# bytedance/DeepSolid

Hardware: AMD Instinct MI355X
Metric: local-energy evals/sec (higher is better)
Workload: dtype f64; 1 GPU; bcc_li 24 e- (12,12), total_energy primal (E_kin forward-Laplacian + Ewald), default detnet ((256,32),)*3, 8 dets; batch_per_gpu=4096, global_batch=4096, parallelism=walker-dp1

## Files before the change

### deepsolid_amd/_lib.py

```python
import ctypes as C
import os

_HERE = os.path.dirname(os.path.abspath(__file__))
LIB_PATH = os.environ.get('DEEPSOLID_HIP_LIB') or os.path.join(_HERE, 'libdeepsolid_hip.so')

DS_MAX_LAYERS = 8
DS_MAX_SYM = 6
_PD = C.POINTER(C.c_double)


class SystemDesc(C.Structure):
    _fields_ = [
        ('dtype', C.c_int32), ('n_up', C.c_int32), ('n_dn', C.c_int32), ('n_atoms_prim', C.c_int32),
        ('prim_atoms', _PD), ('prim_a', C.c_double * 9), ('sim_a', C.c_double * 9), ('n_sym', C.c_int32),
        ('prim_AV', C.c_double * (DS_MAX_SYM * 3)), ('prim_BV', C.c_double * (DS_MAX_SYM * 3)),
        ('sim_AV', C.c_double * (DS_MAX_SYM * 3)), ('sim_BV', C.c_double * (DS_MAX_SYM * 3)),
        ('n_layers', C.c_int32), ('hidden_single', C.c_int32 * DS_MAX_LAYERS),
        ('hidden_double', C.c_int32 * DS_MAX_LAYERS), ('n_det', C.c_int32), ('distance_type', C.c_int32),
        ('envelope_type', C.c_int32), ('full_det', C.c_int32), ('use_last_layer', C.c_int32),
        ('bias_orbitals', C.c_int32), ('klist_up', _PD), ('klist_dn', _PD),
        ('n_atoms_sim', C.c_int32), ('sim_atoms', _PD), ('sim_charges', _PD), ('dist_mode', C.c_int32),
        ('n_g', C.c_int32), ('gpoints', _PD), ('gweight', _PD), ('ion_exp_re', _PD), ('ion_exp_im', _PD),
        ('ewald_alpha', C.c_double), ('ee_const', C.c_double), ('ei_const', C.c_double), ('ii_total', C.c_double),
    ]
# ... 16 lines not shown
        ('shell_l', _PI), ('shell_nprim', _PI), ('exps', _PD), ('coefs', _PD), ('n_k', C.c_int32), ('kpts', _PD),
        ('n_images', C.c_int32), ('images', _PD), ('n_up', C.c_int32), ('n_dn', C.c_int32), ('nocc_up', _PI), ('nocc_dn', _PI),
        ('mo_up', _PD), ('mo_dn', _PD),
    ]


class EcpDesc(C.Structure):
    _PI = C.POINTER(C.c_int32)
    _fields_ = [
        ('a', C.c_double * 9), ('n_atoms', C.c_int32), ('atoms', _PD), ('atom_species', _PI), ('n_species', C.c_int32),
        ('n_l', _PI), ('r_cut_loc', _PD), ('r_cut_nl', _PD), ('term_offset', _PI), ('term_n', _PI), ('term_zeta', _PD),
        ('term_c', _PD), ('n_quad', C.c_int32),
    ]


_VP = C.c_void_p


def _dmc_step_sig(n_lead, n_noise, n_out, ecp):
    step = [C.c_int64, C.c_int] + [C.c_double] * 5 + [C.c_int, C.c_int, C.c_uint64, C.c_uint64]
    return (C.c_int, [_VP] * n_lead + step + [_VP] * n_noise + ([C.c_int64] if ecp else []) + [C.c_int] + [_VP] * n_out +
            ([C.POINTER(C.c_int)] if ecp else []) + [_VP, C.c_int64, _VP])


SIGNATURES = {
    'ds_device_widths': (C.c_int, [C.POINTER(C.c_int32), C.POINTER(C.c_int32), C.c_int32, C.c_int32, C.c_int32, C.c_int32,
                                   C.POINTER(C.c_int32), C.POINTER(C.c_int32), C.POINTER(C.c_int32), C.POINTER(C.c_int32)]),
    'ds_system_create': (C.c_int, [C.POINTER(SystemDesc), C.POINTER(_VP)]),
    'ds_system_destroy': (None, [_VP]),
    'ds_last_error': (C.c_char_p, []),
    'ds_param_count': (C.c_int64, [_VP]),
    'ds_int8_layers': (C.c_int, [_VP]),
    'ds_pair_recompute_layers': (C.c_int, [_VP, C.c_int]),
    'ds_param_layout': (C.c_int, [_VP, C.POINTER(ParamBlock), C.c_int]),
    'ds_workspace_bytes': (C.c_int64, [_VP, C.c_int64]),
    'ds_logpsi': (C.c_int, [_VP, _VP, _VP, C.c_int64, _VP, _VP, _VP, C.c_int64, _VP]),
    'ds_logpsi_grad': (C.c_int, [_VP, _VP, _VP, C.c_int64, _VP, _VP, _VP, _VP, C.c_int64, _VP]),
    'ds_vjp_workspace_bytes': (C.c_int64, [_VP, C.c_int64]),
    'ds_logpsi_vjp': (C.c_int, [_VP, _VP, _VP, C.c_int64, _VP, _VP, _VP, _VP, _VP, C.c_int64, _VP]),
    'ds_pretrain_workspace_bytes': (C.c_int64, [_VP, C.c_int64]),
    'ds_pretrain_loss_vjp': (C.c_int, [_VP, _VP, _VP, C.c_int64, _VP, _VP, _VP, _VP, _VP, C.c_int64, _VP]),
    'ds_kfac_block_count': (C.c_int, [_VP]),
    'ds_kfac_layout': (C.c_int, [_VP, C.POINTER(KfacBlock), C.c_int]),
    'ds_kfac_workspace_bytes': (C.c_int64, [_VP, C.c_int64]),
    'ds_kfac_factors': (C.c_int, [_VP, _VP, _VP, C.c_int64, _VP, _VP, _VP, C.c_int64, _VP]),
    'ds_kfac_step_workspace_bytes': (C.c_int64, [_VP]),
    'ds_kfac_inverses': (C.c_int, [_VP, _VP, C.c_double, C.c_double, _VP, _VP, C.c_int64, _VP]),
    'ds_kfac_precondition': (C.c_int, [_VP, _VP, _VP, _VP, _VP, _VP, C.c_int64, _VP]),
    'ds_kfac_inverses_sized_workspace_bytes': (C.c_int64, [C.c_int, C.POINTER(C.c_int32), C.POINTER(C.c_int32)]),
    'ds_kfac_inverses_sized': (C.c_int, [C.c_int, C.c_int, C.POINTER(C.c_int32), C.POINTER(C.c_int32), C.POINTER(C.c_int32), _VP,
                                        C.c_double, C.c_double, _VP, _VP, C.c_int64, _VP]),
    'ds_jacobian_workspace_bytes': (C.c_int64, [_VP, C.c_int64]),
    'ds_logpsi_jacobian': (C.c_int, [_VP, _VP, _VP, C.c_int64, _VP, C.c_int64, _VP, _VP, _VP, C.c_int64, _VP]),
    'ds_minsr_gram_workspace_bytes': (C.c_int64, [C.c_int64, C.c_int64]),
    'ds_minsr_gram': (C.c_int, [C.c_int, _VP, C.c_int64, C.c_int64, C.c_int64, _VP, _VP, C.c_int64, _VP]),
    'ds_minsr_matvec_workspace_bytes': (C.c_int64, [C.c_int, C.c_int64, C.c_int64]),
    'ds_minsr_matvec': (C.c_int, [C.c_int, C.c_int, _VP, C.c_int64, C.c_int64, C.c_int64, _VP, _VP, _VP, C.c_int64, _VP]),
    'ds_minsr_solve_workspace_bytes': (C.c_int64, [C.c_int64, C.c_int64]),
    'ds_minsr_solve': (C.c_int, [C.c_int64, C.c_int64, C.c_double, C.c_double, _VP, _VP, _VP, _VP, C.c_int64, _VP]),
    'ds_orbitals': (C.c_int, [_VP, _VP, _VP, C.c_int64, _VP, _VP, _VP, C.c_int64, _VP]),
    'ds_ewald': (C.c_int, [_VP, _VP, C.c_int64, _VP, _VP]),
    'ds_local_energy': (C.c_int, [_VP, _VP, _VP, C.c_int64, _VP, _VP, _VP, _VP, _VP, C.c_int64, _VP]),
    'ds_enforce_pbc': (C.c_int, [_PD, C.c_int, _VP, C.c_int64, _VP, _VP, _VP]),
    'ds_observables_workspace_bytes': (C.c_int64, [C.c_int64, C.c_int]),
    'ds_observables': (C.c_int, [_PD, C.c_int, _VP, C.c_int64, C.c_int64, C.POINTER(C.c_int32), C.c_int, C.c_int, _VP, _VP,
                                 C.c_int64, _VP]),
# ... 86 lines not shown
```

### deepsolid_amd/csrc/ds_api.hip

```cpp
#include <cstdarg>

#include "ds_host.h"
#include "ds_tiles.h"

namespace ds {
#define DS_DECL(p) const TileOps<double>* tile_ops_f64_p##p(int); const TileOps<float>* tile_ops_f32_p##p(int);
DS_DECL(0) DS_DECL(1) DS_DECL(2) DS_DECL(3) DS_DECL(4)
#undef DS_DECL
template <> const TileOps<double>* tile_ops<double>(int st) {
    const TileOps<double>* (*parts[])(int) = {tile_ops_f64_p0, tile_ops_f64_p1, tile_ops_f64_p2, tile_ops_f64_p3, tile_ops_f64_p4};
    for (auto f : parts)
        if (const TileOps<double>* o = f(st)) return o;
    return nullptr;
}
template <> const TileOps<float>* tile_ops<float>(int st) {
    const TileOps<float>* (*parts[])(int) = {tile_ops_f32_p0, tile_ops_f32_p1, tile_ops_f32_p2, tile_ops_f32_p3, tile_ops_f32_p4};
    for (auto f : parts)
        if (const TileOps<float>* o = f(st)) return o;
    return nullptr;
}
}

namespace ds {
namespace host {
// ... 309 lines not shown
        hipMemcpy(s->blob32, h32.data(), h32.size() * sizeof(float), hipMemcpyHostToDevice) != hipSuccess) {
        ds_system_destroy(s);
        return fail("upload of the system tables failed");
    }
    relocate<double>(s->sd, (const double*)s->blob64);
    relocate<float>(s->sf, (const float*)s->blob32);
    build_layouts(s);
    {
        int h1max = 0;
        for (int l = 0; l <= s->sd.n_layers; ++l) h1max = std::max(h1max, s->sd.h1[l]);
        if (hipMalloc(&s->lr_w0t, (size_t)h1max * 64 * sizeof(double)) != hipSuccess) {
            ds_system_destroy(s);
            return fail("hipMalloc of the low-rank layer's weight table failed");
        }
    }
    {
        hipDeviceProp_t prop;
        int devid = 0;
        if (hipGetDevice(&devid) == hipSuccess && hipGetDeviceProperties(&prop, devid) == hipSuccess && prop.multiProcessorCount > 0)
            s->n_cu = prop.multiProcessorCount;
    }
    if (hipMalloc((void**)&s->clk_dev, 1024 * sizeof(unsigned long long)) != hipSuccess ||
        hipMemset(s->clk_dev, 0, 1024 * sizeof(unsigned long long)) != hipSuccess) {
        ds_system_destroy(s);
        return fail("hipMalloc of the clock-probe counters failed");
    }
    s->det_valu = getenv("DS_DET_VALU") != nullptr;
    if (const char* e = getenv("DS_VAL_NB")) { const int v = atoi(e); s->val_nb = (v == 1 || v == 2 || v == 4) ? v : 0; }
    s->no_lu_wave = getenv("DS_NO_LU_WAVE") != nullptr;
    s->use_lr = getenv("DS_NO_LOWRANK") == nullptr;
    s->use_pm_skip = getenv("DS_NO_PM_SKIP") == nullptr;
    s->use_pair_expand = getenv("DS_NO_PAIR_EXPAND") == nullptr;
    s->use_pair_recompute = getenv("DS_NO_PAIR_RECOMPUTE") == nullptr;
    s->use_g4 = getenv("DS_NO_G4") == nullptr;
    s->use_i8 = getenv("DS_I8") != nullptr && getenv("DS_NO_I8") == nullptr;
    s->use_ldsb = getenv("DS_NO_LDSB") == nullptr;
    s->use_pair_fuse = getenv("DS_NO_PAIR_FUSE") == nullptr;
    s->use_i8_val = getenv("DS_NO_I8_VAL") == nullptr;
    for (int l = 0; l < DS_MAX_LAYERS; ++l) s->i8_prepped[l] = ~(uint64_t)0;
    if (const char* e = getenv("DS_I8_VAL_MIN_TILES")) s->val_i8_min_tiles = atoll(e);
    if (const char* e = getenv("DS_DBG")) s->dbg = atoi(e);
    s->use_wide = getenv("DS_NO_WIDE") == nullptr;
    s->wide_all = getenv("DS_WIDE_ALL") != nullptr;
    {
        const size_t bytes = i8_planes_bytes(s);
        if (bytes && hipMalloc(&s->i8_wp, bytes) != hipSuccess) {
            ds_system_destroy(s);
            return fail("hipMalloc of the int8 layer's weight planes failed");
        }
    }
    if (const char* e = getenv("DS_CHUNK_WALKERS")) s->chunk_cap = std::min<int64_t>(65535, std::max<int64_t>(1, atol(e)));
    *out = s;
    return 0;
}

void ds_system_destroy(ds_system* s) {
    if (!s) return;
    if (s->clk_dev) (void)hipFree(s->clk_dev);
    if (s->lr_w0t) (void)hipFree(s->lr_w0t);
    if (s->i8_wp) (void)hipFree(s->i8_wp);
    if (s->blob64) (void)hipFree(s->blob64);
    if (s->blob32) (void)hipFree(s->blob32);
    delete s;
}

int64_t ds_param_count(const ds_system* s) { return s ? s->nparams : -1; }
// ... 100 lines not shown
```

### deepsolid_amd/csrc/ds_chain.hip

```cpp
#include "ds_host.h"
#include "ds_tiles.h"

namespace ds {
namespace host {

template <typename T> inline unsigned m2_split(int K2, int N) {
    unsigned z = 1;
    while (z < 8 && K2 % (2 * z) == 0 && (size_t)(K2 / z) * 5 * N * sizeof(T) > 8192) z *= 2;
    return z;
}

enum Stop { STOP_NONE = 0, STOP_G0, STOP_G1, STOP_G2, STOP_G3, STOP_H2_0, STOP_H2_1, STOP_H2_2, STOP_MEAN0, STOP_Q,
            STOP_MOUT, STOP_MINV, STOP_DETS, STOP_TR };

template <typename T> struct DumpReq { int stop; T* out; int64_t cap; int64_t written; };

template <typename T>
int copy_out(DumpReq<T>* dr, const T* src, size_t n, hipStream_t st) {
    size_t m = std::min<size_t>(n, (size_t)dr->cap);
    HIP_OK(hipMemcpyAsync(dr->out, src, m * sizeof(T), hipMemcpyDeviceToDevice, st));
    dr->written = (int64_t)m;
    return 0;
}

enum class LayerKind {
    Dense,
    DenseRes,
    L0Stats,
    L0Epi9Means,
    LowRank1,
    Int8
};
struct PairPlan {
    bool res, res_sep;
    bool expand;
    bool write_out;
    unsigned xz; int EW, NW; size_t xlds;
    bool recompute_prev;
};
struct LayerPlan {
    LayerKind kind;
    bool res_sep;
    bool wide;
    bool pm_mask;
    bool pm_unwritten;
    int prof_kind;
    PairPlan pair;
};
enum class OrbKind { Orb3, Wide, Ldsb, Gemm };
template <typename T> struct ChainPlan {
    const ds::TileOps<T>* to;
    bool lr_on;
    int lr_nc;
    int g4;
    LayerPlan layer[DS_MAX_LAYERS];
    OrbKind orb[2];
    int count(LayerKind k, int n_layers) const {
        int n = 0;
        for (int l = 0; l < n_layers; ++l) n += layer[l].kind == k ? 1 : 0;
        return n;
    }
};

template <typename T>
int plan_chain(const ds_system* s, bool dump, ChainPlan<T>* p) {
    const ds::SysDev<double>& S = s->sd;
    const ds::TileOps<T>* to = p->to = ds::tile_ops<T>(S.P / 16);
    if (!to) return fail("no kernel instance for %d slot tiles (N = %d electrons)", S.P / 16, S.N);
    const int ST = to->ST;
    const bool wide = s->use_wide && to->gemm_wide != nullptr;
    auto gemm_wide = [&](int epi) { return wide && (s->wide_all || ds::gemm_wide_faster<T>(epi)); };
    const int K0loc = S.h1[0] + S.nch * S.h2[0], K0sh = S.nch * S.h1[0];
    p->lr_nc = std::max(2, (K0loc + K0sh + 4 + 15) / 16);
    p->lr_on = !dump && s->use_lr && S.n_layers >= 2 && !s->res1[0] && p->lr_nc <= 4 && S.h1[1] % 16 == 0 && (S.nch * S.h2[1]) % 4 == 0 &&
               3 * (K0loc + K0sh + 4) <= S.h1[1] && p->lr_nc * S.h1[1] < (S.h1[1] - K0loc - K0sh - 4) * ST;
    const int used = S.D - 16 * (ST - 1);
    p->g4 = !s->use_g4 ? 0 : (ST == 5 && used > 8 && used <= 12) ? 3 : (ST == 10 && used <= 4) ? 1 : 0;
    auto pair_geom = [&](PairPlan& pp, int K2o) {
        pp.xz = (!pp.res && K2o == 32) ? 2 : 1;
        pp.EW = (pp.write_out && S.N % 16 == 8 && pp.xz == 2) ? 2 : 1;
        pp.NW = (pp.EW * S.N + 15) / 16;
        pp.xlds = ((size_t)(K2o / pp.xz) * 5 * pp.EW * S.N + (size_t)pp.EW * S.nch * (K2o / pp.xz) * 5) * sizeof(T);
    };
    for (int l = 0; l < S.n_layers; ++l) {
        const int Kh = S.h1[l], K2 = S.h2[l], Nout = S.h1[l + 1], Kloc = Kh + S.nch * K2;
        LayerPlan& lp = p->layer[l];
        lp = LayerPlan{};
        if (Nout % 64 || Nout > 1024) return fail("hidden_single must be a multiple of 64 and <= 1024 (got %d)", Nout);
        if (l < S.n_double) {
            PairPlan& pp = lp.pair;
            const int K2o = S.h2[l + 1];
            if (K2o != 32 && K2o != 16) return fail("hidden_double must be 16 or 32 (got %d)", K2o);
            if (K2 % 4) return fail("pair-stream width %d is not a multiple of 4", K2);
            pp.res_sep = s->res2[l] && l == 0;
            pp.res = s->res2[l] && !pp.res_sep;
            pp.write_out = l + 1 < S.n_double || s->use_last;
            pair_geom(pp, K2o);
            pp.expand = !dump && s->use_pair_expand && !pp.res_sep && l + 1 < S.n_layers && pp.NW <= 8 && pp.xlds <= 150 * 1024;
            if (l >= 1) {
                PairPlan& prev = p->layer[l - 1].pair;
                pp.recompute_prev = sizeof(T) == 8 && !dump && s->use_pair_recompute && pp.res && pp.expand && S.h2[l - 1] <= 8 &&
                                    !prev.res && !prev.res_sep && prev.expand;
                if (pp.recompute_prev) {
                    prev.write_out = false;
                    pair_geom(prev, K2);
                }
            }
        }
        const bool res = s->res1[l];
        lp.res_sep = res && l == 0 && (Kloc % 16 != 0 || S.nf * S.A != Nout);
// ... 19 lines not shown
        lp.pm_unwritten = !dump && l >= 1 && !lp.wide &&
                          (lp.kind == LayerKind::LowRank1 ? s->use_pm_skip : (lp.pm_mask && ds::pm_instance<T>(ST)));
    }
    const int Korb = S.h1[S.n_layers] + (s->use_last ? S.nch * S.h2[S.n_layers] : 0);
    if (Korb % 16) return fail("orbital head with K = %d: the GEMM's operand ring needs K %% 16 == 0", Korb);
    for (int sp = 0; sp < S.nch; ++sp) {
        const int OC = S.ocols[sp];
        if (to->gemm_orb3 && OC % 256 != 0 && OC % 192 == 0) p->orb[sp] = OrbKind::Orb3;
        else if (gemm_wide(5)) p->orb[sp] = OrbKind::Wide;
        else if (to->orbital_lb && s->use_ldsb && OC % 64 == 0) p->orb[sp] = OrbKind::Ldsb;
        else p->orb[sp] = OrbKind::Gemm;
    }
    return 0;
}

template <typename T>
int run_chain(ds_system* s, const T* params, const T* x, int64_t Bc, Arena<T> ws, hipStream_t st, T* out_ke, T* out_logabs,
              T* out_phase, DumpReq<T>* dr, T* out_grad = nullptr) {
    const ds::SysDev<T>& S = dev<T>(s);
    const WsLayout& L = s->ws;
    const Carve<T> c = carve<T>(s, ws, Bc);
    if (!ws.ok) return carve_fail("forward-Laplacian chain");
    auto blk = [&](int i) { return params + s->blocks[i].offset; };
    const int stop = dr ? dr->stop : STOP_NONE;
    ChainPlan<T> plan;
    if (int rc = plan_chain<T>(s, dr != nullptr, &plan)) return rc;
    const ds::TileOps<T>* to = plan.to;
    const int NB = to->NB, ST = to->ST, lr_nc = plan.lr_nc;
    const bool lr_on = plan.lr_on;
    const int K0loc = S.h1[0] + S.nch * S.h2[0], K0sh = S.nch * S.h1[0];
    {
        ProfScope ps(s, DS_PROF_FEATURES, st);
        size_t sh = (size_t)(9 * S.N) * sizeof(T) + (size_t)S.N * S.A * S.nf * sizeof(ds::Jet5<T>);
        hipLaunchKernelGGL((ds::k_features<T>), dim3((unsigned)Bc), dim3(256), sh, st, S, x, blk(s->i_pi[0]), blk(s->i_sg[0]),
                           blk(s->i_pi[S.nch - 1]), blk(s->i_sg[S.nch - 1]), lr_on ? c.XL : c.G[0], lr_on ? K0loc : S.ldk, c.MEAN[0], c.H2[0], c.Q);
    }
    if (lr_on) {
        const int n = S.h1[1] * 16 * lr_nc;
        hipLaunchKernelGGL((ds::k_lr_w0t<T>), dim3((unsigned)((n + 255) / 256)), dim3(256), 0, st, blk(s->i_wloc[0]), blk(s->i_wsh[0]), K0loc, K0sh,
                           S.h1[1], 16 * lr_nc, (T*)s->lr_w0t);
    }
    if (stop == STOP_MEAN0) return copy_out(dr, c.MEAN[0], (size_t)S.nch * S.h1[0] * S.P * Bc, st);
    if (stop == STOP_H2_0) return copy_out(dr, c.H2[0], (size_t)S.h2[0] * 5 * S.NP * Bc, st);
    if (stop == STOP_Q) return copy_out(dr, c.Q, L.Q * Bc, st);
    int gi = 0, hi = 0;
    for (int l = 0; l < S.n_layers; ++l) {
        const LayerPlan& lp = plan.layer[l];
        const int Kh = S.h1[l], K2 = S.h2[l], Nout = S.h1[l + 1];
        if (!(l > 0 && plan.layer[l - 1].pair.expand)) {
            ProfScope ps(s, DS_PROF_M2_EXPAND, st);
            const bool xl = lr_on && l == 0;
            hipLaunchKernelGGL((ds::k_m2_expand<T>), dim3(S.N, (unsigned)Bc, m2_split<T>(K2, S.N)), dim3(256), (size_t)(K2 * 5 * S.N + S.nch * K2 * 5) / m2_split<T>(K2, S.N) * sizeof(T), st, S,
                               c.H2[hi], K2, xl ? c.XL : c.G[gi], Kh, xl ? K0loc : S.ldk, lp.pm_unwritten ? 1 : 0);
        }
        if (stop == STOP_G0 + l) return copy_out(dr, c.G[gi], L.G * Bc, st);
        if (l < S.n_double) {
            const PairPlan& pp = lp.pair;
            const int K2o = S.h2[l + 1];
            const T* W2 = blk(s->i_w2[l]); const T* b2 = blk(s->i_b2[l]);
            ProfScope ps(s, DS_PROF_TWO_LAYER, st);
            if (pp.expand) {
#define DS_TWOX(NT2, RES) hipLaunchKernelGGL((ds::k_two_layer_expand<T, NT2, RES>), dim3(S.N / pp.EW, (unsigned)Bc, pp.xz), dim3(64 * pp.NW), pp.xlds, st, S, c.H2[hi], K2, W2, b2, \
                                             pp.write_out ? c.H2[hi ^ 1] : (T*)nullptr, c.G[gi ^ 1], S.h1[l + 1], S.ldk, plan.layer[l + 1].pm_unwritten ? 1 : 0, pp.EW)
#define DS_TWOXP(NT2) hipLaunchKernelGGL((ds::k_two_layer_expand<T, NT2, true, true>), dim3(S.N / pp.EW, (unsigned)Bc, pp.xz), dim3(64 * pp.NW), pp.xlds, st, S, c.H2[hi ^ 1], S.h2[l - 1], W2, b2, \
                                         pp.write_out ? c.H2[hi] : (T*)nullptr, c.G[gi ^ 1], S.h1[l + 1], S.ldk, plan.layer[l + 1].pm_unwritten ? 1 : 0, pp.EW,               \
                                         blk(s->i_w2[l - 1]), blk(s->i_b2[l - 1]))
                if (pp.recompute_prev) {
                    if constexpr (sizeof(T) == 8) { if (K2o == 32) DS_TWOXP(2); else DS_TWOXP(1); }
                } else if (K2o == 32 && pp.res) DS_TWOX(2, true);
                else if (pp.res) DS_TWOX(1, true);
                else DS_TWOX(1, false);
#undef DS_TWOXP
#undef DS_TWOX
            } else {
                const dim3 grid((S.NP / 16 + 3) / 4, (unsigned)Bc);
#define DS_TWO(NT2, RES) hipLaunchKernelGGL((ds::k_two_layer<T, NT2, RES, false>), grid, dim3(256), 0, st, S, c.H2[hi], K2, W2, b2, c.H2[hi ^ 1])
                if (K2o == 32) { if (pp.res) DS_TWO(2, true); else DS_TWO(2, false); }
                else { if (pp.res) DS_TWO(1, true); else DS_TWO(1, false); }
#undef DS_TWO
            }
            if (pp.res_sep)
                launch_pair_res_add<T>(dim3((unsigned)(((size_t)K2o * 5 * S.NP + 255) / 256), (unsigned)Bc), st, c.H2[hi], K2, c.H2[hi ^ 1], K2o, S.nf, S.NP);
// ... 207 lines not shown

template <typename T> void ewald_triple(ds_system* s, const void* x, int64_t B, void* out, hipStream_t st) {
    const ds::SysDev<T>& S = dev<T>(s);
    size_t sh = ds::ewald_lds_bytes(S);
    hipLaunchKernelGGL((ds::k_ewald<T>), dim3((unsigned)B), dim3(256), sh, st, S, (const T*)x, (T*)out);
}

template <typename T>
int64_t debug_stage_impl(ds_system* s, const void* params, const void* x, int64_t B, int stop, void* out, int64_t out_elems, void* ws,
                         int64_t ws_bytes, hipStream_t st) {
    DumpReq<T> dr{stop, (T*)out, out_elems, 0};
    const int rc = run_chain<T>(s, (const T*)params, (const T*)x, B, arena_of<T>(ws, ws_bytes), st, nullptr, nullptr, nullptr, &dr);
    return rc ? -1 : dr.written;
}

int logpsi_grad_forward(ds_system* s, const void* params, const void* x, int64_t B, void* out_logabs, void* out_phase, void* out_grad,
                        void* ws, int64_t ws_bytes, hipStream_t st) {
    return DS_BY_DTYPE(s->dtype, logpsi_grad_impl, s, params, x, B, out_logabs, out_phase, out_grad, ws, ws_bytes, st);
}

int int8_energy_layers(const ds_system* s, bool dump) {
    ChainPlan<double> plan;
    return plan_chain<double>(s, dump, &plan) == 0 ? plan.count(LayerKind::Int8, s->sd.n_layers) : 0;
}

template <typename T> int pair_recompute_count(const ds_system* s, bool dump) {
    ChainPlan<T> plan;
    if (plan_chain<T>(s, dump, &plan)) return 0;
    int n = 0;
    for (int l = 0; l < s->sd.n_double && l < s->sd.n_layers; ++l) n += plan.layer[l].pair.recompute_prev ? 1 : 0;
    return n;
}

template <typename T> void launch_pair_res_add(dim3 grid, hipStream_t st, const T* Hin, int Kin, T* Hout, int Kout, int n_res, int NP) {
    hipLaunchKernelGGL((ds::k_pair_res_add<T>), grid, dim3(256), 0, st, Hin, Kin, Hout, Kout, n_res, NP);
}

template <typename T>
void launch_layer_res_add(dim3 grid, hipStream_t st, const T* Xin, size_t x_ws, size_t x_ts, T* Gout, size_t g_ws, size_t g_ts, int n_res,
                          int Nout, int P) {
    hipLaunchKernelGGL((ds::k_layer_res_add<T>), grid, dim3(256), 0, st, Xin, x_ws, x_ts, Gout, g_ws, g_ts, n_res, Nout, P);
}

#define DS_INST(T)                                                                                      \
    template void launch_pair_res_add<T>(dim3, hipStream_t, const T*, int, T*, int, int, int);          \
    template void launch_layer_res_add<T>(dim3, hipStream_t, const T*, size_t, size_t, T*, size_t, size_t, int, int, int);
DS_INST(double) DS_INST(float)
#undef DS_INST

}
}

using namespace ds::host;

extern "C" {

int ds_int8_layers(const ds_system* s) {
    if (!s) return -1;
    return int8_energy_layers(s, false);
}

int ds_pair_recompute_layers(const ds_system* s, int dump) {
    if (!s) return -1;
    return s->dtype == 0 ? pair_recompute_count<double>(s, dump != 0) : pair_recompute_count<float>(s, dump != 0);
}

int ds_local_energy(ds_system* s, const void* params, const void* x, int64_t B, void* out_ke, void* out_ewald, void* out_logabs,
                    void* out_phase, void* ws, int64_t ws_bytes, void* stream) {
    if (s) ++s->call_seq;
    if (!s || !params || !x || !ws) return fail("null argument");
    if (B <= 0) return 0;
    hipStream_t st = (hipStream_t)stream;
    return DS_BY_DTYPE(s->dtype, local_energy_impl, s, params, x, B, out_ke, out_ewald, out_logabs, out_phase, ws, ws_bytes, st);
}

int ds_logpsi_grad(ds_system* s, const void* params, const void* x, int64_t B, void* out_logabs, void* out_phase, void* out_grad,
                   void* ws, int64_t ws_bytes, void* stream) {
    if (s) ++s->call_seq;
    if (!s || !params || !x || !ws || !out_grad) return fail("null argument");
    if (B <= 0) return 0;
    hipStream_t st = (hipStream_t)stream;
    return logpsi_grad_forward(s, params, x, B, out_logabs, out_phase, out_grad, ws, ws_bytes, st);
}

int ds_ewald(ds_system* s, const void* x, int64_t B, void* out, void* stream) {
    if (!s || !x || !out) return fail("null argument");
    if (B <= 0) return 0;
    hipStream_t st = (hipStream_t)stream;
    DS_BY_DTYPE(s->dtype, ewald_triple, s, x, B, out, st);
    HIP_OK(hipGetLastError());
    return 0;
}

int64_t ds_debug_stage(ds_system* s, const void* params, const void* x, int64_t B, const char* stage, void* out, int64_t out_elems,
                       void* ws, int64_t ws_bytes, void* stream) {
    if (s) ++s->call_seq;
    if (!s || !params || !x || !stage || !out || !ws) { fail("null argument"); return -1; }
// ... 17 lines not shown
```

### deepsolid_amd/csrc/ds_host.h

```cpp
#pragma once
#include "ds_base.h"
#include "ds_value.h"

namespace ds {
namespace host {

template <typename I> inline I rup(I x, int m) { return (x + m - 1) / m * m; }

template <typename T> struct Arena {
    T* base = nullptr;
    size_t cap = SIZE_MAX, used = 0;
    bool ok = true;
    T* take(size_t n) { T* p = base ? base + used : nullptr; used += n; ok = ok && used <= cap; return p; }
    void align(size_t k) { take((k - used % k) % k); }
    template <typename F> void part(T* buf, size_t n, F&& carve) { Arena a{buf, n}; carve(a); ok = ok && a.ok; }
};
template <typename T> Arena<T> arena_of(void* ws, int64_t ws_bytes) { return Arena<T>{(T*)ws, (size_t)std::max<int64_t>(ws_bytes, 0) / sizeof(T)}; }
template <typename F> size_t measure(F&& layout) { Arena<double> a; layout(a); return a.used; }

struct PassSize { size_t fixed, per_group; };
inline int64_t groups_per_pass(int64_t B, int64_t esz, const PassSize& z, int64_t budget) {
    const int64_t groups = std::min<int64_t>((std::max<int64_t>(B, 1) + ds::PV - 1) / ds::PV, 64);
    return std::max<int64_t>(1, std::min<int64_t>(groups, budget / ((int64_t)z.per_group * esz)));
}
// ... 7 lines not shown
    size_t G, MEAN, ZB, H2, Q, MOUT, MINV, DETS, TR;
    size_t PARTM = 0;
    size_t XL = 0;
    size_t YO = 0;
    size_t mout_off[2], minv_off[2], dets_off[2], tr_off[2];
    size_t per_walker;
};

}
}

struct ds_system {
    ds_system_desc d;
    int dtype;
    ds::SysDev<double> sd;
    ds::SysDev<float> sf;
    void* blob64 = nullptr;
    void* blob32 = nullptr;
    std::vector<ds_param_block> blocks;
    int64_t nparams = 0;
    ds::host::WsLayout ws;
    ds::host::WsLayout wsv;
    std::vector<int> i_wloc, i_wsh, i_b, i_w2, i_b2, i_worb, i_wsh_orb, i_borb, i_pi, i_sg;
    bool use_last = false;
    int32_t ref_single[DS_MAX_LAYERS] = {0}, ref_double[DS_MAX_LAYERS] = {0};
    bool res1[DS_MAX_LAYERS] = {false}, res2[DS_MAX_LAYERS] = {false};
    bool no_lu_wave = false;
    int val_nb = 0;
    bool det_valu = false;
    int64_t chunk_cap = 4096;
    bool use_g4 = true;
    bool use_pair_expand = true;
    bool use_pair_recompute = true;
    bool use_pm_skip = true;
    bool use_lr = true;
    void* lr_w0t = nullptr;
    int64_t val_i8_min_tiles = 512;
    bool use_i8_val = true;
    bool use_pair_fuse = true;
    bool use_ldsb = true;
    bool use_i8 = false;
    void* i8_wp = nullptr;
    uint64_t call_seq = 0;
    uint64_t i8_prepped[DS_MAX_LAYERS];
    int n_cu = 256;
    bool use_wide = true;
    bool wide_all = false;
    int dbg = 0;
    bool prof_on = false;
    int prof_only = -1;
    std::vector<std::pair<hipEvent_t, hipEvent_t>> prof_ev[DS_PROF_KINDS];
    std::vector<hipEvent_t> prof_pool;
    unsigned long long* clk_dev = nullptr;
    bool prof_failed = false;
};

namespace ds {
namespace host {

struct ProfScope {
    ds_system* s; int kind; hipStream_t st; hipEvent_t e0 = nullptr, e1 = nullptr;
    static hipEvent_t get(ds_system* s) {
        if (!s->prof_pool.empty()) { hipEvent_t e = s->prof_pool.back(); s->prof_pool.pop_back(); return e; }
        hipEvent_t e = nullptr;
        if (hipEventCreate(&e) != hipSuccess) { s->prof_failed = true; return nullptr; }
        return e;
// ... 165 lines not shown
```

### deepsolid_amd/csrc/ds_kernels.h

```cpp
#pragma once
#include "ds_device.h"

namespace ds {

#define DS_MAXL 8

template <typename T> struct SysDev {
    int N, n_up, n_dn, A, L, K, nch;
    int D, P, NP;
    int n_layers, n_double;
    int h1[DS_MAXL + 1];
    int h2[DS_MAXL + 1];
    int ldk;
    int full_det, env_type, bias_orb;
    int dist_type, nf;
    int norb[2];
    int n_detch;
    int det_n[2];
    int mat_ch[2], row_off[2];
    int nparam[2];
    int nparam_max;
    int ocols[2];
    const T *prim_a, *prim_ainv, *sim_a, *sim_ainv, *prim_AV, *prim_BV, *sim_AV, *sim_BV, *atoms;
    const T* klist[2];
// ... 156 lines not shown
        T v = 0;
        for (int j = j0; j < j0 + ns; ++j) v += hs[kc * N + j];
        sums[idx] = v / T(ns);
    }
    __syncthreads();
    T* Ge = G + ((size_t)(w * N + e) * ldg + row0 + k0) * P;
    typedef T vec4 __attribute__((ext_vector_type(4)));
    const int QP = P / 4;
    for (int idx = tid; idx < S.nch * Kc * QP; idx += nt) {
        const int row = idx / QP, sq = idx - row * QP, k = row % Kc, s = row / Kc;
        const int j0 = s == 0 ? 0 : S.n_up, ns = s == 0 ? S.n_up : S.n_dn;
        if (skip) {
            const int t = sq >> 2, lo = (2 + 3 * j0) >> 4, hi = (4 + 3 * (j0 + ns - 1)) >> 4;
            if (!(t == 0 || t == ((2 + 3 * e) >> 4) || t == ((4 + 3 * e) >> 4) || (t >= lo && t <= hi))) continue;
        }
        const T inv = T(1) / T(ns);
        const T* sm = sums + (s * Kc + k) * 5;
        vec4 v;
#pragma unroll
        for (int u = 0; u < 4; ++u) {
            const int slot = 4 * sq + u;
            T x = 0;
            if (slot == 0) x = sm[0];
            else if (slot == 1) x = sm[4];
            else if (slot < S.D) {
                const int j = (slot - 2) / 3, c = (slot - 2) - 3 * j;
                if (j == e) x = -sm[1 + c];
                else if (j >= j0 && j < j0 + ns) x = hs[(k * 5 + 1 + c) * N + j] * inv;
            }
            v[u] = x;
        }
        *reinterpret_cast<vec4*>(Ge + ((size_t)s * K2 + k) * P + 4 * sq) = v;
    }
}

template <typename T>
__global__ void __launch_bounds__(256) k_layer_res_add(const T* __restrict__ Xin, size_t x_ws, size_t x_ts, T* __restrict__ Gout, size_t g_ws,
                                                       size_t g_ts, int n_res, int Nout, int P) {
    const T* xi = Xin + (size_t)blockIdx.y * x_ws + (size_t)blockIdx.x * x_ts;
    T* go = Gout + (size_t)blockIdx.y * g_ws + (size_t)blockIdx.x * g_ts;
    const T rs2 = T(0.70710678118654752440);
    for (int idx = threadIdx.x; idx < Nout * P; idx += blockDim.x) {
        const T r = idx < n_res * P ? xi[idx] : T(0);
        go[idx] = (r + go[idx]) * rs2;
    }
}

template <typename T>
__global__ void __launch_bounds__(256) k_pair_res_add(const T* __restrict__ Hin, int Kin, T* __restrict__ Hout, int Kout, int n_res, int NP) {
    const size_t idx = (size_t)blockIdx.x * blockDim.x + threadIdx.x;
    if (idx >= (size_t)Kout * 5 * NP) return;
    const T* hi = Hin + (size_t)blockIdx.y * Kin * 5 * NP;
    T* ho = Hout + (size_t)blockIdx.y * Kout * 5 * NP;
    const T r = idx < (size_t)n_res * 5 * NP ? hi[idx] : T(0);
    ho[idx] = (r + ho[idx]) * T(0.70710678118654752440);
}

constexpr int PM_SLOTS = 3;
template <typename T>
__device__ __forceinline__ void pair_tanh_jet(T z0, T z1, T z2, T z3, T z4, T (&o)[5]) {
    const T y = ds_tanh(z0), d1 = 1 - y * y, d2 = -2 * y * d1;
    o[0] = y; o[1] = d1 * z1; o[2] = d1 * z2; o[3] = d1 * z3;
    o[4] = d1 * z4 + d2 * 2 * (z1 * z1 + z2 * z2 + z3 * z3);
}
__device__ __forceinline__ double as_loaded(double x) { asm("" : "+v"(x)); return x; }
template <typename T, int NT2, bool RES, bool VAL>
// ... 1198 lines not shown
```

### deepsolid_amd/device.py

```python
import ctypes as C
import re
from typing import NamedTuple

import numpy as np
import torch

from . import _lib
from .params import ParamMap

_DTYPES = {torch.float64: 0, torch.float32: 1}


def _pd(a):
    return a.ctypes.data_as(C.POINTER(C.c_double))


def _ptr(t):
    return C.c_void_p(t.data_ptr()) if t is not None else C.c_void_p(0)


def _stream():
    return C.c_void_p(torch.cuda.current_stream().cuda_stream)


# ... 786 lines not shown
            if rc != 0 and attempt == 0:
                m = re.search(r'pair capacity exceeded: the walkers have (\d+) pairs', self.lib.ds_last_error().decode())
                if m:
                    cap = int(m.group(1))
                    continue
            _lib.check(rc, 'ds_ecp_energy')
            break
        return dict(e_loc=energy[:, 0], e_nl=torch.complex(energy[:, 1], energy[:, 2]), pairs=pairs if want_pairs else None,
                    rotations=rot, pair_capacity=cap,
                    ratios=torch.view_as_complex(ratios)[:int(pairs.sum()) * ecp.n_quad] if want_ratios else None)

    def energy_stats(self, ke, ew):
        out = torch.empty(8, dtype=torch.float64, device=self.device)
        _lib.check(self.lib.ds_energy_stats(self.handle, _ptr(ke), _ptr(ew), ke.shape[0], _ptr(out), _stream()), 'ds_energy_stats')
        return out

    def profile(self, on=True, only=None):
        mode = 0 if not on else (1 if only is None else 2 + _lib.PROF_KINDS.index(only))
        _lib.check(self.lib.ds_profile_enable(self.handle, mode), 'ds_profile_enable')

    def profile_read(self):
        n = len(_lib.PROF_KINDS)
        ms = (C.c_double * n)()
        cnt = (C.c_int64 * n)()
        _lib.check(self.lib.ds_profile_read(self.handle, ms, cnt), 'ds_profile_read')
        return {k: (float(ms[i]), int(cnt[i])) for i, k in enumerate(_lib.PROF_KINDS)}

    def int8_layers(self):
        return int(self.lib.ds_int8_layers(self.handle))

    def pair_recompute_layers(self, dump=False):
        return int(self.lib.ds_pair_recompute_layers(self.handle, 1 if dump else 0))

    def profile_clock(self):
        cyc, ticks = C.c_double(0), C.c_double(0)
        _lib.check(self.lib.ds_profile_read_clock(self.handle, C.byref(cyc), C.byref(ticks)), 'ds_profile_read_clock')
        return cyc.value, ticks.value, (cyc.value / ticks.value * 0.1 if ticks.value > 0 else None)

    def debug_stage(self, params, x, stage, n_elems):
        x = self._check_x(x)
        p = self.pack_params(params)
        ws = self.workspace(x.shape[0])
        out = torch.zeros(int(n_elems), dtype=self.dtype, device=self.device)
        n = self.lib.ds_debug_stage(self.handle, _ptr(p), _ptr(x), x.shape[0], stage.encode(), _ptr(out), out.numel(),
                                    _ptr(ws), ws.numel(), _stream())
        if n < 0:
            raise RuntimeError(f'ds_debug_stage({stage}): {self.lib.ds_last_error().decode()}')
        return out[:n]


def observable_sums(recvec, x, q_int, pol_direction):
    _require_gpu()
    if not x.is_cuda:
        raise RuntimeError('observable_sums: walkers must live on the ROCm device (no CPU path)')
    if x.dtype not in _DTYPES:
        raise TypeError(f'observable_sums: walkers must be float64 or float32, got {x.dtype}')
    if x.dim() != 2 or x.shape[1] % 3:
        raise ValueError(f'observable_sums: walkers must have shape (B, 3N), got {tuple(x.shape)}')
    if x.shape[0] < 1:
        raise ValueError('observable_sums: empty walker batch (the observables are batch means)')
    lib = _lib.load()
    x = x.contiguous()
    rv = np.ascontiguousarray(np.asarray(recvec, dtype=np.float64).reshape(3, 3))
    q = np.ascontiguousarray(np.asarray(q_int, dtype=np.int32).reshape(-1, 3))
    B, n_q = x.shape[0], q.shape[0]
    need = lib.ds_observables_workspace_bytes(B, n_q)
# ... 228 lines not shown
```

### include/deepsolid_hip.h

```cpp
#ifndef DEEPSOLID_HIP_H
#define DEEPSOLID_HIP_H

#include <stddef.h>
#include <stdint.h>

#ifdef __cplusplus
extern "C" {
#endif

#define DS_MAX_LAYERS 8
#define DS_MAX_SYM 6

typedef struct ds_system ds_system;

typedef struct ds_system_desc {
    int32_t dtype;
    int32_t n_up, n_dn;
    int32_t n_atoms_prim;
    const double* prim_atoms;
    double prim_a[9];
    double sim_a[9];
    int32_t n_sym;
    double prim_AV[DS_MAX_SYM * 3], prim_BV[DS_MAX_SYM * 3];
    double sim_AV[DS_MAX_SYM * 3], sim_BV[DS_MAX_SYM * 3];
// ... 10 lines not shown
    const double* klist_dn;
    int32_t n_atoms_sim;
    const double* sim_atoms;
    const double* sim_charges;
    int32_t dist_mode;
    int32_t n_g;
    const double* gpoints;
    const double* gweight;
    const double* ion_exp_re;
    const double* ion_exp_im;
    double ewald_alpha;
    double ee_const;
    double ei_const;
    double ii_total;
} ds_system_desc;

typedef struct ds_param_block {
    int64_t offset;
    int32_t rows, cols;
} ds_param_block;

int ds_device_widths(const int32_t* hidden_single, const int32_t* hidden_double, int32_t n_layers, int32_t n_in_single,
                     int32_t n_in_double, int32_t n_double, int32_t* dev_single, int32_t* dev_double, int32_t* res_single,
                     int32_t* res_double);

int ds_system_create(const ds_system_desc* desc, ds_system** out);
void ds_system_destroy(ds_system* sys);
const char* ds_last_error(void);

int ds_int8_layers(const ds_system* sys);

int ds_pair_recompute_layers(const ds_system* sys, int dump);

int64_t ds_param_count(const ds_system* sys);
int ds_param_layout(const ds_system* sys, ds_param_block* blocks, int max_blocks);

int64_t ds_workspace_bytes(const ds_system* sys, int64_t B);

int ds_logpsi(ds_system* sys, const void* params, const void* x, int64_t B,
              void* out_logabs, void* out_phase, void* ws, int64_t ws_bytes, void* stream);

int ds_logpsi_grad(ds_system* sys, const void* params, const void* x, int64_t B,
                   void* out_logabs, void* out_phase, void* out_grad, void* ws, int64_t ws_bytes, void* stream);

int64_t ds_vjp_workspace_bytes(const ds_system* sys, int64_t B);
int ds_logpsi_vjp(ds_system* sys, const void* params, const void* x, int64_t B, const void* cot, void* grad,
                  void* out_logabs, void* out_phase, void* ws, int64_t ws_bytes, void* stream);

int64_t ds_pretrain_workspace_bytes(const ds_system* sys, int64_t B);
int ds_pretrain_loss_vjp(ds_system* sys, const void* params, const void* x, int64_t B, const void* target_up,
                         const void* target_dn, void* out_loss, void* grad, void* ws, int64_t ws_bytes, void* stream);

typedef struct ds_kfac_block {
    int32_t kind, index;
    int32_t n_param_blocks;
    int32_t param_blocks[3];
    int32_t has_bias, d_in, d_out, repeats;
    int64_t a_offset, g_offset;
} ds_kfac_block;
int ds_kfac_block_count(const ds_system* sys);
int ds_kfac_layout(const ds_system* sys, ds_kfac_block* blocks, int max_blocks);
int64_t ds_kfac_workspace_bytes(const ds_system* sys, int64_t B);
int ds_kfac_factors(ds_system* sys, const void* params, const void* x, int64_t B, void* factors, void* grad_seed, void* ws,
                    int64_t ws_bytes, void* stream);

int64_t ds_kfac_step_workspace_bytes(const ds_system* sys);
// ... 206 lines not shown
```

Before: 69700 local-energy evals/s.

## Fuse layer-0 pair-mean expansion into the features kernel for f64

Adds a templated features kernel that, besides the one-electron features, envelope Q and means, computes pair distance jets chunk by chunk in LDS and writes the layer-0 pair-mean columns of G directly. This lets the separate k_m2_expand launch for layer 0 be skipped, which removes a kernel launch and a reread of H2 from global memory. The fused kernel uses a larger shared-memory footprint, up to 64 KB, and serializes over electron chunks inside one block, which may lower occupancy. It is on by default for f64 and can be disabled with an environment variable.

```diff
diff --git a/deepsolid_amd/_lib.py b/deepsolid_amd/_lib.py
--- a/deepsolid_amd/_lib.py
+++ b/deepsolid_amd/_lib.py
@@ -72,6 +72,7 @@
     'ds_param_count': (C.c_int64, [_VP]),
     'ds_int8_layers': (C.c_int, [_VP]),
     'ds_pair_recompute_layers': (C.c_int, [_VP, C.c_int]),
+    'ds_features_fused': (C.c_int, [_VP, C.c_int]),
     'ds_param_layout': (C.c_int, [_VP, C.POINTER(ParamBlock), C.c_int]),
     'ds_workspace_bytes': (C.c_int64, [_VP, C.c_int64]),
     'ds_logpsi': (C.c_int, [_VP, _VP, _VP, C.c_int64, _VP, _VP, _VP, C.c_int64, _VP]),
diff --git a/deepsolid_amd/csrc/ds_api.hip b/deepsolid_amd/csrc/ds_api.hip
--- a/deepsolid_amd/csrc/ds_api.hip
+++ b/deepsolid_amd/csrc/ds_api.hip
@@ -365,6 +365,7 @@
     s->use_pm_skip = getenv("DS_NO_PM_SKIP") == nullptr;
     s->use_pair_expand = getenv("DS_NO_PAIR_EXPAND") == nullptr;
     s->use_pair_recompute = getenv("DS_NO_PAIR_RECOMPUTE") == nullptr;
+    s->use_feat_fuse = getenv("DS_NO_FEAT_FUSE") == nullptr;
     s->use_g4 = getenv("DS_NO_G4") == nullptr;
     s->use_i8 = getenv("DS_I8") != nullptr && getenv("DS_NO_I8") == nullptr;
     s->use_ldsb = getenv("DS_NO_LDSB") == nullptr;
diff --git a/deepsolid_amd/csrc/ds_chain.hip b/deepsolid_amd/csrc/ds_chain.hip
--- a/deepsolid_amd/csrc/ds_chain.hip
+++ b/deepsolid_amd/csrc/ds_chain.hip
@@ -53,6 +53,8 @@
     bool lr_on;
     int lr_nc;
     int g4;
+    bool feat_fuse;
+    int feat_ec, feat_ulen; size_t feat_lds;
     LayerPlan layer[DS_MAX_LAYERS];
     OrbKind orb[2];
     int count(LayerKind k, int n_layers) const {
@@ -76,6 +78,8 @@
                3 * (K0loc + K0sh + 4) <= S.h1[1] && p->lr_nc * S.h1[1] < (S.h1[1] - K0loc - K0sh - 4) * ST;
     const int used = S.D - 16 * (ST - 1);
     p->g4 = !s->use_g4 ? 0 : (ST == 5 && used > 8 && used <= 12) ? 3 : (ST == 10 && used <= 4) ? 1 : 0;
+    p->feat_lds = ds::features_pm_lds<T>(S.N, S.A, S.nf, S.nch, S.h2[0], &p->feat_ec, &p->feat_ulen);
+    p->feat_fuse = sizeof(T) == 8 && s->use_feat_fuse && S.n_layers >= 1 && p->feat_lds <= 64 * 1024;
     auto pair_geom = [&](PairPlan& pp, int K2o) {
         pp.xz = (!pp.res && K2o == 32) ? 2 : 1;
         pp.EW = (pp.write_out && S.N % 16 == 8 && pp.xz == 2) ? 2 : 1;
@@ -161,8 +165,16 @@
     {
         ProfScope ps(s, DS_PROF_FEATURES, st);
         size_t sh = (size_t)(9 * S.N) * sizeof(T) + (size_t)S.N * S.A * S.nf * sizeof(ds::Jet5<T>);
-        hipLaunchKernelGGL((ds::k_features<T>), dim3((unsigned)Bc), dim3(256), sh, st, S, x, blk(s->i_pi[0]), blk(s->i_sg[0]),
-                           blk(s->i_pi[S.nch - 1]), blk(s->i_sg[S.nch - 1]), lr_on ? c.XL : c.G[0], lr_on ? K0loc : S.ldk, c.MEAN[0], c.H2[0], c.Q);
+#define DS_FEATPM(DT) hipLaunchKernelGGL((ds::k_features<T, DT>), dim3((unsigned)Bc), dim3(256), plan.feat_lds, st, S, x, blk(s->i_pi[0]), blk(s->i_sg[0]), \
+                                      blk(s->i_pi[S.nch - 1]), blk(s->i_sg[S.nch - 1]), lr_on ? c.XL : c.G[0], lr_on ? K0loc : S.ldk, c.MEAN[0], c.H2[0], c.Q,    \
+                                      plan.feat_ec, plan.feat_ulen, plan.layer[0].pm_unwritten ? 1 : 0)
+        if (plan.feat_fuse) {
+            if constexpr (sizeof(T) == 8) { if (S.dist_type == 0) DS_FEATPM(0); else DS_FEATPM(1); }
+        } else {
+            hipLaunchKernelGGL((ds::k_features<T>), dim3((unsigned)Bc), dim3(256), sh, st, S, x, blk(s->i_pi[0]), blk(s->i_sg[0]),
+                               blk(s->i_pi[S.nch - 1]), blk(s->i_sg[S.nch - 1]), lr_on ? c.XL : c.G[0], lr_on ? K0loc : S.ldk, c.MEAN[0], c.H2[0], c.Q);
+        }
+#undef DS_FEATPM
     }
     if (lr_on) {
         const int n = S.h1[1] * 16 * lr_nc;
@@ -176,7 +188,7 @@
     for (int l = 0; l < S.n_layers; ++l) {
         const LayerPlan& lp = plan.layer[l];
         const int Kh = S.h1[l], K2 = S.h2[l], Nout = S.h1[l + 1];
-        if (!(l > 0 && plan.layer[l - 1].pair.expand)) {
+        if (!(l > 0 && plan.layer[l - 1].pair.expand) && !(l == 0 && plan.feat_fuse)) {
             ProfScope ps(s, DS_PROF_M2_EXPAND, st);
             const bool xl = lr_on && l == 0;
             hipLaunchKernelGGL((ds::k_m2_expand<T>), dim3(S.N, (unsigned)Bc, m2_split<T>(K2, S.N)), dim3(256), (size_t)(K2 * 5 * S.N + S.nch * K2 * 5) / m2_split<T>(K2, S.N) * sizeof(T), st, S,
@@ -450,6 +462,11 @@
     return n;
 }
 
+template <typename T> int features_fused(const ds_system* s, bool dump) {
+    ChainPlan<T> plan;
+    return plan_chain<T>(s, dump, &plan) == 0 && plan.feat_fuse ? 1 : 0;
+}
+
 template <typename T> void launch_pair_res_add(dim3 grid, hipStream_t st, const T* Hin, int Kin, T* Hout, int Kout, int n_res, int NP) {
     hipLaunchKernelGGL((ds::k_pair_res_add<T>), grid, dim3(256), 0, st, Hin, Kin, Hout, Kout, n_res, NP);
 }
@@ -481,6 +498,11 @@
 int ds_pair_recompute_layers(const ds_system* s, int dump) {
     if (!s) return -1;
     return s->dtype == 0 ? pair_recompute_count<double>(s, dump != 0) : pair_recompute_count<float>(s, dump != 0);
+}
+
+int ds_features_fused(const ds_system* s, int dump) {
+    if (!s) return -1;
+    return s->dtype == 0 ? features_fused<double>(s, dump != 0) : features_fused<float>(s, dump != 0);
 }
 
 int ds_local_energy(ds_system* s, const void* params, const void* x, int64_t B, void* out_ke, void* out_ewald, void* out_logabs,
diff --git a/deepsolid_amd/csrc/ds_host.h b/deepsolid_amd/csrc/ds_host.h
--- a/deepsolid_amd/csrc/ds_host.h
+++ b/deepsolid_amd/csrc/ds_host.h
@@ -63,6 +63,7 @@
     bool use_g4 = true;
     bool use_pair_expand = true;
     bool use_pair_recompute = true;
+    bool use_feat_fuse = true;
     bool use_pm_skip = true;
     bool use_lr = true;
     void* lr_w0t = nullptr;
diff --git a/deepsolid_amd/csrc/ds_kernels.h b/deepsolid_amd/csrc/ds_kernels.h
--- a/deepsolid_amd/csrc/ds_kernels.h
+++ b/deepsolid_amd/csrc/ds_kernels.h
@@ -212,6 +212,221 @@
         }
         *reinterpret_cast<vec4*>(Ge + ((size_t)s * K2 + k) * P + 4 * sq) = v;
     }
+}
+
+template <typename T, int DT>
+__global__ void __launch_bounds__(256) k_features(SysDev<T> S, const T* __restrict__ x, const T* __restrict__ env_pi0,
+                                                     const T* __restrict__ env_sg0, const T* __restrict__ env_pi1,
+                                                     const T* __restrict__ env_sg1, T* __restrict__ G, int ldg, T* __restrict__ MEAN,
+                                                     T* __restrict__ H2, T* __restrict__ Q, int EC, int ulen, int skip) {
+    extern __shared__ __attribute__((aligned(16))) char smem_raw[];
+    typedef T vec4 __attribute__((ext_vector_type(4)));
+    typedef T vec2 __attribute__((ext_vector_type(2)));
+    const int w = blockIdx.x, tid = threadIdx.x, nt = blockDim.x;
+    const int N = S.N, A = S.A, P = S.P, NP = S.NP, nf = S.nf, nch = S.nch, L = S.L;
+    T* xs = reinterpret_cast<T*>(smem_raw);
+    T* px = xs + 3 * N;
+    T* sx = px + 3 * N;
+    T* un = sx + 3 * N + ((3 * N) & 1);
+    int* qok = reinterpret_cast<int*>(un + ulen);
+    Jet5<T>* jea = reinterpret_cast<Jet5<T>*>(qok + 256);
+    const T* xw = x + (size_t)w * 3 * N;
+    for (int i = tid; i < N; i += nt) {
+        T r[3] = {xw[3 * i], xw[3 * i + 1], xw[3 * i + 2]}, o[3], wr[3];
+        for (int c = 0; c < 3; ++c) xs[3 * i + c] = r[c];
+        wrap_point(r, S.prim_a, S.prim_ainv, o, wr);
+        for (int c = 0; c < 3; ++c) px[3 * i + c] = o[c];
+        wrap_point(r, S.sim_a, S.sim_ainv, o, wr);
+        for (int c = 0; c < 3; ++c) sx[3 * i + c] = o[c];
+    }
+    __syncthreads();
+    for (int ia = tid; ia < N * A; ia += nt) {
+        const int i = ia / A, a = ia % A;
+        T r[3];
+        for (int c = 0; c < 3; ++c) r[c] = px[3 * i + c] - S.atoms[3 * a + c];
+        Jet5<T> o[7];
+        if constexpr (DT == 0) nu_distance_jet(r, S.prim_AV, S.prim_BV, L, o); else tri_distance_jet(r, S.prim_AV, S.prim_BV, L, o);
+#pragma unroll
+        for (int f = 0; f < 7; ++f)
+            if (f < nf) jea[nf * ia + f] = o[f];
+    }
+    __syncthreads();
+    const int K1 = S.h1[0], QP = P / 4;
+    T* Gw = G + (size_t)w * N * ldg * P;
+    for (int idx = tid; idx < N * K1 * QP; idx += nt) {
+        const int rw = idx / QP, sq = idx - rw * QP, i = rw / K1, k = rw - i * K1;
+        vec4 v = {0, 0, 0, 0};
+        if (k < nf * A) {
+            const Jet5<T>& j = jea[nf * (i * A + k / nf) + (k % nf)];
+            const int lo = 2 + 3 * i;
+#pragma unroll
+            for (int u = 0; u < 4; ++u) {
+                const int slot = 4 * sq + u;
+                if (slot == 0) v[u] = j.v;
+                else if (slot == 1) v[u] = j.l;
+                else if (slot >= lo && slot < lo + 3) v[u] = j.g[slot - lo];
+            }
+        }
+        *reinterpret_cast<vec4*>(Gw + ((size_t)i * ldg + k) * P + 4 * sq) = v;
+    }
+    T* Mw = MEAN + (size_t)w * nch * K1 * P;
+    for (int idx = tid; idx < nch * K1 * QP; idx += nt) {
+        const int rw = idx / QP, sq = idx - rw * QP, s = rw / K1, k = rw - s * K1;
+        const int i0 = s == 0 ? 0 : S.n_up, ns = s == 0 ? S.n_up : S.n_dn;
+        const int a = k / nf, f = k % nf;
+        vec4 o;
+#pragma unroll
+        for (int u = 0; u < 4; ++u) {
+            const int slot = 4 * sq + u;
+            T v = 0;
+            if (k < nf * A) {
+                if (slot < 2) {
+                    for (int i = i0; i < i0 + ns; ++i) v += (slot == 0 ? jea[nf * (i * A + a) + f].v : jea[nf * (i * A + a) + f].l);
+                } else if (slot < S.D) {
+                    const int j = (slot - 2) / 3;
+                    if (j >= i0 && j < i0 + ns) v = jea[nf * (j * A + a) + f].g[(slot - 2) % 3];
+                }
+            }
+            o[u] = v / T(ns);
+        }
+        *reinterpret_cast<vec4*>(Mw + (size_t)rw * P + 4 * sq) = o;
+    }
+    T* Qw = Q + (size_t)w * N * S.nparam_max * 10;
+    const int nq = N * S.nparam_max;
+    for (int c0 = 0; c0 < nq; c0 += 256) {
+        const int idx = c0 + tid;
+        const int i = idx / S.nparam_max, p = idx - i * S.nparam_max;
+        const int s = spin_of(i, S.n_up);
+        const bool on = tid < 256 && idx < nq && p < S.nparam[s];
+        if (tid < 256) qok[tid] = on ? 1 : 0;
+        if (on) {
+            const T* pi_ = s == 0 ? env_pi0 : env_pi1;
+            const T* sg_ = s == 0 ? env_sg0 : env_sg1;
+            const int np = S.nparam[s];
+            Jet5<T> e = jet_zero<T>();
+            for (int a = 0; a < A; ++a) {
+                const T pw = pi_[a * np + p];
+                if (S.env_type == 0) {
+                    const Jet5<T>& sd = jea[nf * (i * A + a)];
+                    const T sg = sg_[a * np + p];
+                    const T u = sd.v * sg;
+                    const T ex = pw * ds_exp(-ds_abs(u));
+                    e = jet_add(e, jet_fn(sd, ex, -ds_sign(u) * sg * ex, sg * sg * ex));
+                } else {
+                    Jet5<T> r2 = jet_zero<T>();
+                    for (int m = 0; m < 3; ++m) {
+                        Jet5<T> u = jet_zero<T>();
+                        if (S.env_type == 1) u = jet_scale(sg_[(a * 3 + m) * np + p], jea[nf * (i * A + a) + 1 + m]);
+                        else
+                            for (int k = 0; k < 3; ++k) u = jet_add(u, jet_scale(sg_[((k * 3 + m) * A + a) * np + p], jea[nf * (i * A + a) + 1 + k]));
+                        r2 = jet_add(r2, jet_mul(u, u));
+                    }
+                    const T r = ds_sqrt(r2.v);
+                    const Jet5<T> rj = jet_fn(r2, r, T(0.5) / r, T(-0.25) / (r * r2.v));
+                    const T ex = pw * ds_exp(-r);
+                    e = jet_add(e, jet_fn(rj, ex, -ex, ex));
+                }
+            }
+            const int m = p % S.norb[s];
+            const T* kv = S.klist[s] + 3 * m;
+            const T kx = kv[0] * xs[3 * i] + kv[1] * xs[3 * i + 1] + kv[2] * xs[3 * i + 2];
+            T sn, cs;
+            ds_sincos(kx, &sn, &cs);
+            const T k2 = kv[0] * kv[0] + kv[1] * kv[1] + kv[2] * kv[2];
+            T* q = un + tid * 10;
+            q[0] = e.v * cs; q[1] = e.v * sn;
+            T lre = e.l * cs - e.v * k2 * cs, lim = e.l * sn - e.v * k2 * sn;
+            for (int c = 0; c < 3; ++c) {
+                q[2 + 2 * c] = e.g[c] * cs - e.v * kv[c] * sn;
+                q[3 + 2 * c] = e.g[c] * sn + e.v * kv[c] * cs;
+                lre += 2 * e.g[c] * (-kv[c] * sn);
+                lim += 2 * e.g[c] * (kv[c] * cs);
+            }
+            q[8] = lre; q[9] = lim;
+        }
+        __syncthreads();
+        const int cnt = min(256, nq - c0);
+        for (int v = tid; v < 5 * cnt; v += nt)
+            if (qok[v / 5]) *reinterpret_cast<vec2*>(Qw + (size_t)c0 * 10 + 2 * v) = *reinterpret_cast<const vec2*>(un + 2 * v);
+        __syncthreads();
+    }
+    const int K2 = S.h2[0], ECN = EC * N;
+    T* Hw = H2 + (size_t)w * K2 * 5 * NP;
+    T* hs = un;
+    T* sums = un + K2 * 5 * ECN;
+    for (int idx = tid; idx < K2 * 5 * (NP - N * N); idx += nt) {
+        const int r = idx / (NP - N * N);
+        Hw[(size_t)r * NP + N * N + (idx - r * (NP - N * N))] = 0;
+    }
+    for (int e0 = 0; e0 < N; e0 += EC) {
+        const int ne = min(EC, N - e0);
+        for (int lp = tid; lp < ne * N; lp += nt) {
+            const int el = lp / N, j = lp - el * N, e = e0 + el;
+            Jet5<T> o[8];
+#pragma unroll
+            for (int f = 0; f < 8; ++f) o[f] = jet_zero<T>();
+            if (e != j) {
+                T r[3];
+                for (int c = 0; c < 3; ++c) r[c] = sx[3 * j + c] - sx[3 * e + c];
+                if constexpr (DT == 0) nu_distance_jet(r, S.sim_AV, S.sim_BV, L, o); else tri_distance_jet(r, S.sim_AV, S.sim_BV, L, o);
+            }
+#pragma unroll
+            for (int f = 0; f < 8; ++f) {
+                if (f >= K2) break;
+                hs[(f * 5 + 0) * ECN + lp] = o[f].v;
+                hs[(f * 5 + 1) * ECN + lp] = o[f].g[0];
+                hs[(f * 5 + 2) * ECN + lp] = o[f].g[1];
+                hs[(f * 5 + 3) * ECN + lp] = o[f].g[2];
+                hs[(f * 5 + 4) * ECN + lp] = 2 * o[f].l;
+            }
+        }
+        __syncthreads();
+        for (int idx = tid; idx < K2 * 5 * ne * N; idx += nt) {
+            const int r = idx / (ne * N), lp = idx - r * (ne * N);
+            Hw[(size_t)r * NP + e0 * N + lp] = hs[r * ECN + lp];
+        }
+        for (int idx = tid; idx < ne * nch * K2 * 5; idx += nt) {
+            const int el = idx / (nch * K2 * 5), r = idx - el * (nch * K2 * 5), s = r / (5 * K2), kc = r - s * (5 * K2);
+            const int j0 = s == 0 ? 0 : S.n_up, ns = s == 0 ? S.n_up : S.n_dn;
+            T v = 0;
+            for (int j = j0; j < j0 + ns; ++j) v += hs[kc * ECN + el * N + j];
+            sums[idx] = v / T(ns);
+        }
+        __syncthreads();
+        for (int idx = tid; idx < ne * nch * K2 * QP; idx += nt) {
+            const int rw = idx / QP, sq = idx - rw * QP, el = rw / (nch * K2), r = rw - el * (nch * K2), s = r / K2, k = r - s * K2;
+            const int e = e0 + el;
+            const int j0 = s == 0 ? 0 : S.n_up, ns = s == 0 ? S.n_up : S.n_dn;
+            if (skip) {
+                const int t = sq >> 2, lo = (2 + 3 * j0) >> 4, hi = (4 + 3 * (j0 + ns - 1)) >> 4;
+                if (!(t == 0 || t == ((2 + 3 * e) >> 4) || t == ((4 + 3 * e) >> 4) || (t >= lo && t <= hi))) continue;
+            }
+            const T inv = T(1) / T(ns);
+            const T* sm = sums + ((el * nch + s) * K2 + k) * 5;
+            vec4 v;
+#pragma unroll
+            for (int u = 0; u < 4; ++u) {
+                const int slot = 4 * sq + u;
+                T xv = 0;
+                if (slot == 0) xv = sm[0];
+                else if (slot == 1) xv = sm[4];
+                else if (slot < S.D) {
+                    const int j = (slot - 2) / 3, c = (slot - 2) - 3 * j;
+                    if (j == e) xv = -sm[1 + c];
+                    else if (j >= j0 && j < j0 + ns) xv = hs[(k * 5 + 1 + c) * ECN + el * N + j] * inv;
+                }
+                v[u] = xv;
+            }
+            *reinterpret_cast<vec4*>(Gw + ((size_t)e * ldg + K1 + s * K2 + k) * P + 4 * sq) = v;
+        }
+        __syncthreads();
+    }
+}
+template <typename T> inline size_t features_pm_lds(int N, int A, int nf, int nch, int K2, int* EC, int* ulen) {
+    *EC = std::max(1, std::min(N, 2560 / (K2 * 5 * N)));
+    *ulen = std::max(2560, K2 * 5 * *EC * N + 5 * nch * K2 * *EC);
+    *ulen += *ulen & 1;
+    return (size_t)(9 * N + ((3 * N) & 1) + *ulen) * sizeof(T) + 256 * sizeof(int) + (size_t)N * A * nf * sizeof(Jet5<T>);
 }
 
 template <typename T>
diff --git a/deepsolid_amd/device.py b/deepsolid_amd/device.py
--- a/deepsolid_amd/device.py
+++ b/deepsolid_amd/device.py
@@ -842,6 +842,9 @@
     def pair_recompute_layers(self, dump=False):
         return int(self.lib.ds_pair_recompute_layers(self.handle, 1 if dump else 0))
 
+    def features_fused(self, dump=False):
+        return int(self.lib.ds_features_fused(self.handle, 1 if dump else 0))
+
     def profile_clock(self):
         cyc, ticks = C.c_double(0), C.c_double(0)
         _lib.check(self.lib.ds_profile_read_clock(self.handle, C.byref(cyc), C.byref(ticks)), 'ds_profile_read_clock')
diff --git a/include/deepsolid_hip.h b/include/deepsolid_hip.h
--- a/include/deepsolid_hip.h
+++ b/include/deepsolid_hip.h
@@ -66,6 +66,8 @@
 
 int ds_pair_recompute_layers(const ds_system* sys, int dump);
 
+int ds_features_fused(const ds_system* sys, int dump);
+
 int64_t ds_param_count(const ds_system* sys);
 int ds_param_layout(const ds_system* sys, ds_param_block* blocks, int max_blocks);
 
```

Result: no change. 69520 local-energy evals/s (-0.2%).
